# Coolzyh/Globecom2020-ResourceAllocationGNN

Hardware: AMD Instinct MI355X
Metric: graph-instances/sec (fwd+bwd), 20-V2V-link graphs, batch 4096 (higher is better)
Workload: dtype f32; 1 GPU; BASELINE.json configs[1]: 20 V2V links, feat_dim=64, 2-layer GNN, global batch 4096 synthetic graphs cut into 1 shard(s), fit step = fwd+Huber+bwd+Adam; weights=per-node (reference semantics), global_batch=4096, graphs_per_gpu=4096, scaling=strong, n_params=767040, aggregation=edge-bitset-walk, ranks_seen=1, launch=eager, parallelism=dp1

## Files before the change

globecom2020-resourceallocationgnn_amd/csrc/kernels.hpp:

```cpp
#pragma once
#include <hip/hip_runtime.h>
#include <stdint.h>
#include <type_traits>

namespace v2x {

typedef float f32x4 __attribute__((ext_vector_type(4)));
typedef const __attribute__((address_space(1))) float* gfloat_p;
#define V2X_MFMA(a, b, c) __builtin_amdgcn_mfma_f32_16x16x4f32((a), (b), (c), 0, 0, 0)

constexpr int XE = 16;
constexpr int H1 = 80, H2 = 40, H3 = 20;
constexpr int H2P = 48, H3P = 32, CP = 16;
constexpr int LD1 = H1 + 4, LD2 = H2P + 4, LD3 = H3P + 4, LD4 = CP + 4;

struct RowPad { int pad_at, n_pad, k_real; };
__device__ __forceinline__ int real_row(const RowPad& p, int rp) {
  int rr = rp < p.pad_at ? rp : (rp < p.pad_at + p.n_pad ? -1 : rp - p.n_pad);
  return rr < p.k_real ? rr : -1;
}

template <int KP, int NP>
struct WeightImageRegs { float4 v[(KP * (NP / 4) + 255) / 256]; };

// ... 1223 lines not shown
      const int n = col + t;
      df[(((kb * FB + (n >> 4)) * 64) + (n & 15) + 16 * kgp) * 4 + s4] = pv[t];
    }
  }
  if (stage) {
    int ntb = -1;
    if (kp < F) ntb = kp >> 4;
    else if (kp >= F + XE) ntb = FB + ((kp - F - XE) >> 4);
    if (ntb >= 0) {
      float* db = k.bwd + ((int64_t)(stage - 1) * k.S + slot) * (FB * 2 * FB * 256);
      *reinterpret_cast<float4*>(db + ((((col >> 4) * 2 * FB + ntb) * 64) + (kp & 15) + 16 * ((col & 15) >> 2)) * 4) = p;
    }
  }
}

struct AdamArgs {
  AdamPack pack;
  float* param; float* grad; float* mom; float* vel;
  const float* slab; int64_t slab_stride; int n_slabs;
  int n_layers; int64_t layer_end4[16]; int layer_slabs[16];
  int64_t n4;
  float lr_t, beta1, beta2, eps;
  int do_adam;
  int n_adam_blocks;
  const float* rowloss; float* loss; int loss_n_idx, loss_stride; float loss_scale;
  int64_t loss_slot_stride;
  int loss_split; float* loss_part; unsigned* loss_cnt;
  int64_t range_begin4, range_end4;
  int64_t range2_begin4, range2_end4;
  const float* grad_direct;
  int groups;
};

__global__ __launch_bounds__(256) void k_reduce_adam(AdamArgs a) {
  if ((int)blockIdx.x >= a.n_adam_blocks) {
    __shared__ float red[256];
    __shared__ int is_last;
    const int lb = blockIdx.x - a.n_adam_blocks;
    const int slot = lb / a.loss_split, part = lb - slot * a.loss_split;
    const int per = (a.loss_n_idx + a.loss_split - 1) / a.loss_split;
    const int i1 = min((part + 1) * per, a.loss_n_idx);
    float s = 0.f;
    for (int i = part * per + threadIdx.x; i < i1; i += 256) s += a.rowloss[(int64_t)i * a.loss_stride + (int64_t)slot * a.loss_slot_stride];
    red[threadIdx.x] = s;
    __syncthreads();
    for (int o = 128; o > 0; o >>= 1) {
      if ((int)threadIdx.x < o) red[threadIdx.x] += red[threadIdx.x + o];
// ... 7 lines not shown
      __hip_atomic_store(a.loss_part + part, red[0], __ATOMIC_RELAXED, __HIP_MEMORY_SCOPE_AGENT);
      const unsigned ticket = __hip_atomic_fetch_add(a.loss_cnt, 1u, __ATOMIC_ACQ_REL, __HIP_MEMORY_SCOPE_AGENT);
      is_last = ticket == (unsigned)a.loss_split - 1;
      if (is_last) {
        float t = 0.f;
        for (int k = 0; k < a.loss_split; ++k) t += __hip_atomic_load(a.loss_part + k, __ATOMIC_RELAXED, __HIP_MEMORY_SCOPE_AGENT);
        a.loss[slot] = t * a.loss_scale;
        __hip_atomic_store(a.loss_cnt, 0u, __ATOMIC_RELAXED, __HIP_MEMORY_SCOPE_AGENT);
      }
    }
    return;
  }
  __shared__ float4 part[256];
  const int G = a.groups, cols = 256 / G;
  const int col = threadIdx.x % cols, grp = threadIdx.x / cols;
  const int64_t len1 = a.range_end4 - a.range_begin4, len_all = len1 + (a.range2_end4 - a.range2_begin4);
  for (int64_t base = (int64_t)blockIdx.x * cols; base < len_all; base += (int64_t)a.n_adam_blocks * cols) {
    const int64_t t = base + col;
    const bool act = t < len_all;
    const int64_t i = t < len1 ? a.range_begin4 + t : a.range2_begin4 + (t - len1);
    float4 g = make_float4(0.f, 0.f, 0.f, 0.f);
    bool direct = false;
    if (a.slab) {
      if (act) {
        int l = 0;
        while (l + 1 < a.n_layers && i >= a.layer_end4[l]) ++l;
        const int ns = a.layer_slabs[l];
        float4 g1 = make_float4(0.f, 0.f, 0.f, 0.f), g2 = g1, g3 = g1;
        int c = grp;
        for (; c + 3 * G < ns; c += 4 * G) {
          const float4 t0 = reinterpret_cast<const float4*>(a.slab + (int64_t)c * a.slab_stride)[i];
          const float4 t1 = reinterpret_cast<const float4*>(a.slab + (int64_t)(c + G) * a.slab_stride)[i];
          const float4 t2 = reinterpret_cast<const float4*>(a.slab + (int64_t)(c + 2 * G) * a.slab_stride)[i];
          const float4 t3 = reinterpret_cast<const float4*>(a.slab + (int64_t)(c + 3 * G) * a.slab_stride)[i];
          g.x += t0.x; g.y += t0.y; g.z += t0.z; g.w += t0.w;
          g1.x += t1.x; g1.y += t1.y; g1.z += t1.z; g1.w += t1.w;
          g2.x += t2.x; g2.y += t2.y; g2.z += t2.z; g2.w += t2.w;
          g3.x += t3.x; g3.y += t3.y; g3.z += t3.z; g3.w += t3.w;
        }
        for (; c < ns; c += G) {
          const float4 t = reinterpret_cast<const float4*>(a.slab + (int64_t)c * a.slab_stride)[i];
          g.x += t.x; g.y += t.y; g.z += t.z; g.w += t.w;
        }
        g.x = (g.x + g1.x) + (g2.x + g3.x); g.y = (g.y + g1.y) + (g2.y + g3.y);
        g.z = (g.z + g1.z) + (g2.z + g3.z); g.w = (g.w + g1.w) + (g2.w + g3.w);
        if (ns == 0 && grp == 0) g = reinterpret_cast<const float4*>(a.grad_direct)[i];
        direct = ns == 0 && a.grad == a.grad_direct;
      }
      if (G > 1) {
        part[threadIdx.x] = g;
        __syncthreads();
        if (grp == 0) {
          for (int k = 1; k < G; ++k) {
            const float4 t = part[k * cols + col];
            g.x += t.x; g.y += t.y; g.z += t.z; g.w += t.w;
          }
        }
        __syncthreads();
      }
      if (act && grp == 0 && !direct) reinterpret_cast<float4*>(a.grad)[i] = g;
    } else if (act && grp == 0) {
      g = reinterpret_cast<const float4*>(a.grad)[i];
    }
    if (a.do_adam && act && grp == 0) {
      float4 m = reinterpret_cast<float4*>(a.mom)[i], v = reinterpret_cast<float4*>(a.vel)[i];
      float4 p = reinterpret_cast<float4*>(a.param)[i];
      const float b1 = a.beta1, b2 = a.beta2, ob1 = 1.f - a.beta1, ob2 = 1.f - a.beta2;
      m.x = b1 * m.x + ob1 * g.x; m.y = b1 * m.y + ob1 * g.y; m.z = b1 * m.z + ob1 * g.z; m.w = b1 * m.w + ob1 * g.w;
      v.x = b2 * v.x + ob2 * (g.x * g.x); v.y = b2 * v.y + ob2 * (g.y * g.y);
      v.z = b2 * v.z + ob2 * (g.z * g.z); v.w = b2 * v.w + ob2 * (g.w * g.w);
      p.x -= a.lr_t * m.x / (sqrtf(v.x) + a.eps); p.y -= a.lr_t * m.y / (sqrtf(v.y) + a.eps);
      p.z -= a.lr_t * m.z / (sqrtf(v.z) + a.eps); p.w -= a.lr_t * m.w / (sqrtf(v.w) + a.eps);
      reinterpret_cast<float4*>(a.mom)[i] = m;
      reinterpret_cast<float4*>(a.vel)[i] = v;
      reinterpret_cast<float4*>(a.param)[i] = p;
      if (a.pack.fwd) pack_scatter(a.pack, 4 * i, p);
    }
  }
}

__global__ __launch_bounds__(256) void k_zero_rows(float* dst, int64_t slot_stride, int64_t count) {
  float* p = dst + blockIdx.y * slot_stride;
  for (int64_t i = ((int64_t)blockIdx.x * 256 + threadIdx.x) * 4; i < count; i += (int64_t)gridDim.x * 1024)
    *reinterpret_cast<float4*>(p + i) = make_float4(0.f, 0.f, 0.f, 0.f);
}

__global__ __launch_bounds__(256) void k_adam_scalar(float* p, const float* g, float* m, float* v,
// ... 317 lines not shown
```

globecom2020-resourceallocationgnn_amd/csrc/kernels_mlpwg.hpp:

```cpp
#pragma once
#include "kernels.hpp"
#include <type_traits>

namespace v2x {

struct MlpWgLayer { int64_t layer_off, slot_stride; int n_real; RowPad pad; };
struct MlpWgArgs {
  float* slab; int64_t slab_stride; MlpWgLayer l[4];
  int tiles_per_slot, slot_span, tiles_per_wg, n_slots, n_slabs;
  long long* ts;
};
struct MlpTrainWgArgs { MlpArgs a; MlpWgArgs w; };

template <int F>
struct MlpWgLds {
  static constexpr int KB1 = 2 * (F / 16) + 1;
  static constexpr int BLK = 256;
  static constexpr int PER_WAVE = (KB1 + 5 + 5) * BLK;
  static constexpr int STAGE = (MlpLds<F>::TOTAL + 3) / 4 * 4;
  static constexpr int T0 = 0, T1 = KB1 * 5, T2 = T1 + 5 * 3, T3 = T2 + 3 * 2, TILES = T3 + 2;
  static constexpr int NBIAS = (5 + 3 + 2 + 1) * 16;
  static constexpr int TOTAL = STAGE + 4 * PER_WAVE;
  static constexpr int X_SET = TILES * 256;
  static constexpr int X_BIAS = 2 * X_SET;
  static_assert(X_BIAS + 4 * NBIAS <= TOTAL, "accumulator exchange must fit");
};

#define V2X_WAVE_SYNC()                                      \
  do {                                                       \
    __builtin_amdgcn_fence(__ATOMIC_RELEASE, "wavefront");   \
    __builtin_amdgcn_wave_barrier();                         \
    __builtin_amdgcn_fence(__ATOMIC_ACQUIRE, "wavefront");   \
    __builtin_amdgcn_sched_barrier(0);                       \
  } while (0)

#define V2X_DS_ILV(NLD, PER)                                   \
  {                                                            \
    _Pragma("unroll") for (int u_ = 0; u_ < (NLD); ++u_) {     \
      __builtin_amdgcn_sched_group_barrier(0x100, 1, 0);       \
// ... 401 lines not shown
  __syncthreads();
  mark();
  if ((wv & 1) == 0) add(std::false_type{}); else add(std::true_type{});
  const float* bq = sBias4 + min((int)threadIdx.x, G::NBIAS - 1);
  const float bsum4 = (bq[0] + bq[G::NBIAS]) + (bq[2 * G::NBIAS] + bq[3 * G::NBIAS]);
  __syncthreads();
  if (threadIdx.x < G::NBIAS) sBias4[threadIdx.x] = bsum4;
  __syncthreads();
  mark();
  const float* sA = smem;
  const float* sB = smem + G::X_SET;
  const float* sBias = sBias4;
  const int first_wg = tile0 / w.tiles_per_wg;
  const int my_slab = blockIdx.x - first_wg;
  float* slab = w.slab + (int64_t)my_slab * w.slab_stride;
  if constexpr (WG0)
    wg_write<5, H1>(sA + G::T0 * 256, sB + G::T0 * 256, sBias, slab + w.l[0].layer_off + slot * w.l[0].slot_stride, w.l[0]);
  wg_write<3, H2>(sA + G::T1 * 256, sB + G::T1 * 256, sBias + 5 * 16, slab + w.l[1].layer_off + slot * w.l[1].slot_stride, w.l[1]);
  wg_write<2, H3>(sA + G::T2 * 256, sB + G::T2 * 256, sBias + 8 * 16, slab + w.l[2].layer_off + slot * w.l[2].slot_stride, w.l[2]);
  wg_write<1, 0>(sA + G::T3 * 256, sB + G::T3 * 256, sBias + 10 * 16, slab + w.l[3].layer_off + slot * w.l[3].slot_stride, w.l[3]);
  mark();
  if (tsp && tsn < 64) tsp[tsn] = (long long)wall_clock64();
}

}
```

globecom2020-resourceallocationgnn_amd/csrc/knobs.hpp:

```cpp
#pragma once
#include <cstdlib>

namespace v2x {

struct Knobs {
  int fused = 1;
  int fused_compl = 1;
  int fused_split = -1;
  int fused_split_fwd = 1;
  int fused_split_bwd = 1;
  int fused_ts = 0;
  int small_predict = 1;
  int small_pinned = 1;
  int ragged_fused = 1;
  int ragged_fused_bwd = 1;
  int ragged_packed = 1;
  int ragged_plan_fold = 1;
  int ragged_small = 0;
  int frag_handoff = 1;
  int frag_with_dense0_role = 1;
  int mlp_wg0 = -1;
  int mlp_wg0_tiles = 12;
  int dqn_fused_targets = 1;
  int wide_merge = 1;
  int wide_fold = 1;
  int wide_adam = 1;
  int wide_tail = 1;
  int wide_slots = 0;
  int wg_embed_merge = 1;
  int wg_rounds = 0;
  int wg_chunk = 0;
  int wg_chunk_gnn = 0;
  int wg_chunk_dense = 1024;
  int wg_chunk_embed = 0;
  int wg_chunk_d123 = 512;
  int wg_chunk_merged = 0;
  int wg_merged_min_rows = 64;
// ... 17 lines not shown
  num("V2X_FUSED_SPLIT", k.fused_split);
  num("V2X_FUSED_SPLIT_FWD", k.fused_split_fwd);
  num("V2X_FUSED_SPLIT_BWD", k.fused_split_bwd);
  num("V2X_FUSED_TS", k.fused_ts);
  num("V2X_SMALL_PREDICT", k.small_predict);
  num("V2X_SMALL_PINNED", k.small_pinned);
  num("V2X_RAGGED_FUSED", k.ragged_fused);
  num("V2X_RAGGED_FUSED_BWD", k.ragged_fused_bwd);
  num("V2X_RAGGED_PACKED", k.ragged_packed);
  num("V2X_RAGGED_PLAN_FOLD", k.ragged_plan_fold);
  num("V2X_RAGGED_SMALL", k.ragged_small);
  num("V2X_FRAG_HANDOFF", k.frag_handoff);
  num("V2X_FRAG_WITH_DENSE0_ROLE", k.frag_with_dense0_role);
  num("V2X_MLP_WG0", k.mlp_wg0);
  num("V2X_MLP_WG0_TILES", k.mlp_wg0_tiles);
  num("V2X_DQN_FUSED_TARGETS", k.dqn_fused_targets);
  num("V2X_WIDE_MERGE", k.wide_merge);
  num("V2X_WIDE_FOLD", k.wide_fold);
  num("V2X_WIDE_ADAM", k.wide_adam);
  num("V2X_WIDE_TAIL", k.wide_tail);
  num("V2X_WIDE_SLOTS", k.wide_slots);
  num("V2X_WG_EMBED_MERGE", k.wg_embed_merge);
  num("V2X_WG_ROUNDS", k.wg_rounds);
  num("V2X_WG_CHUNK", k.wg_chunk);
  num("V2X_WG_CHUNK_GNN", k.wg_chunk_gnn);
  num("V2X_WG_CHUNK_DENSE", k.wg_chunk_dense);
  num("V2X_WG_CHUNK_EMBED", k.wg_chunk_embed);
  num("V2X_WG_CHUNK_D123", k.wg_chunk_d123);
  num("V2X_WG_CHUNK_MERGED", k.wg_chunk_merged);
  num("V2X_WG_MERGED_MIN_ROWS", k.wg_merged_min_rows);
// ... 19 lines not shown
```

globecom2020-resourceallocationgnn_amd/csrc/v2xgnn.hip:

```cpp
#include "../../include/v2xgnn.h"
#include "kernels.hpp"
#include "kernels_wide.hpp"
#include "kernels_fused.hpp"
#include "kernels_fused_split.hpp"
#include "kernels_mlpwg.hpp"
#include "kernels_small.hpp"
#include "kernels_ragged.hpp"
#include "kernels_ragged_small.hpp"
#include "host_pack.hpp"
#include "knobs.hpp"

#include <hip/hip_runtime.h>
#include <algorithm>
#include <cmath>
#include <cstdio>
#include <cstdlib>
#include <cstring>
#include <map>
#include <mutex>
#include <string>
#include <type_traits>
#include <vector>

using namespace v2x;

namespace {

thread_local std::string g_err;

struct LayerDesc {
  int64_t off;
  int64_t slot_stride;
  int k_real, n_out;
  int kp, np;
  RowPad pad;
  int n_slabs = 0;
};

struct DevBuf {
  void* p = nullptr;
  size_t cap = 0;
};

struct ProfRec { int id; hipEvent_t ev0, ev1; };

struct GraphKey {
  int kind; const void* ptrs[12]; int sizes[6]; double scalar;
  int64_t gen;
  bool operator<(const GraphKey& o) const { return memcmp(this, &o, sizeof(GraphKey)) < 0; }
};

// ... 10 lines not shown
  int64_t iterations = 0;
  int64_t cap_rows = 0;
  std::vector<float*> h, a;
  float *z1 = nullptr, *z2 = nullptr, *z3 = nullptr, *q = nullptr;
  float *dq = nullptr, *dz1 = nullptr, *dz2 = nullptr, *dz3 = nullptr, *gha = nullptr, *rowloss = nullptr;
  std::vector<float*> dpre;
  unsigned* nbmask = nullptr;
  bool frag_live = false;
  unsigned short* gate_bits = nullptr;
  int64_t gate_stride = 0;
  hipStream_t cap = nullptr;
  float* loss_dev = nullptr;
  float* loss_part = nullptr;
  float* zero_buf = nullptr;
  float* slab = nullptr; int slab_cap = 0;
  int reduce_groups = 0;
  std::vector<int32_t> wide_rec_tiles, wide_rec_roles;
  DevBuf st_xe, st_nbr, st_goff, st_rp, st_ci, st_y, st_q;
  DevBuf adj_mask;
  DevBuf plan_buf;
  int plan_len = 0;
  Knobs knobs;
  long long* ts_buf = nullptr;
  bool raw_params = false;
  bool pk_stale = false;
  unsigned long long* small_h = nullptr;
  unsigned long long* small_sync = nullptr;
  char* pin_h = nullptr; char* pin_d = nullptr;
  float *pk_fwd = nullptr, *pk_bwd = nullptr;
  unsigned long long* xchg_buf = nullptr;
  unsigned long long* xchg_sync = nullptr;
  int xchg_cap_tiles = 0;
  int* flag_host = nullptr;
  int* flag_dev = nullptr;
  bool have_fwd = false;
  std::string err;
  bool prof = false;
  std::vector<std::string> prof_names;
  std::vector<ProfRec> prof_recs;
  struct GraphEntry { hipGraphExec_t exec; std::vector<int> n_slabs; bool frag_live; int reduce_groups; };
  int64_t ws_gen = 0;
  std::map<GraphKey, GraphEntry> graphs;
  bool capturing = false;
  float* adam_scal = nullptr;
  bool prof_no_fuse = false;
  hipStream_t dp_st = nullptr;
  std::vector<hipEvent_t> dp_ev;
};

namespace {

#define FAIL(m, code, ...)                                   \
  do {                                                       \
    char _b[512];                                            \
    snprintf(_b, sizeof(_b), __VA_ARGS__);                   \
// ... 191 lines not shown
  } else {
    nc = (n_idx + rows - 1) / rows;
  }
  if (nc < 1) nc = 1;
  const int max_nc = (n_idx + 4 * WG_TR - 1) / (4 * WG_TR);
  if (nc > max_nc) nc = max_nc;
  if (nc < 1) nc = 1;
  int chunk = (n_idx + nc - 1) / nc;
  chunk = (chunk + 4 * WG_TR - 1) / (4 * WG_TR) * (4 * WG_TR);
  nc = (n_idx + chunk - 1) / chunk;
  if (nc < 1) nc = 1;
  *chunk_out = chunk;
  return nc;
}

int ensure_slabs(v2x_model* m, int nc) {
  if (nc <= m->slab_cap) return V2X_OK;
  if (m->capturing) FAIL(m, V2X_ESTATE, "slab growth during graph capture");
  drop_graphs(m);
  if (m->slab) HIPCHK(m, hipFree(m->slab));
  m->slab = nullptr;
  HIPCHK(m, hipMalloc(reinterpret_cast<void**>(&m->slab), (size_t)nc * m->P * sizeof(float)));
  HIPCHK(m, hipMemset(m->slab, 0, (size_t)nc * m->P * sizeof(float)));
  HIPCHK(m, hipDeviceSynchronize());
  m->slab_cap = nc;
  return V2X_OK;
}

struct FlagWord { int* host = nullptr; int* dev = nullptr; };
int alloc_flag(FlagWord* f) {
  void* h = nullptr;
  if (hipHostMalloc(&h, 64, hipHostMallocMapped) != hipSuccess) return V2X_EHIP;
  memset(h, 0, 64);
  void* d = nullptr;
  if (hipHostGetDevicePointer(&d, h, 0) != hipSuccess) { hipHostFree(h); return V2X_EHIP; }
  f->host = (int*)h; f->dev = (int*)d;
  return V2X_OK;
}
// ... 549 lines not shown
  s.n_slabs = gx;
  return s;
}

template <int F>
int launch_mlp_train_wg_f(v2x_model* m, hipStream_t st, const MlpArgs& a, int n_slots, bool wg0) {
  const size_t lds = (size_t)MlpWgLds<F>::TOTAL * 4;
  const MlpWgSplit sp = mlp_wg_split(a.n_idx, n_slots);
  if (sp.n_slabs > m->slab_cap) FAIL(m, V2X_ESTATE, "mlp_train_wg: slabs not pre-sized (%d > %d)", sp.n_slabs, m->slab_cap);
  MlpTrainWgArgs t;
  memset(&t, 0, sizeof(t));
  t.a = a;
  t.w.slab = m->slab; t.w.slab_stride = m->P;
  t.w.tiles_per_slot = sp.tiles_per_slot; t.w.slot_span = sp.slot_span; t.w.tiles_per_wg = sp.tiles_per_wg; t.w.n_slots = n_slots; t.w.n_slabs = sp.n_slabs;
  t.w.ts = m->ts_buf ? m->ts_buf + 2 * 8 * 64 : nullptr;
  for (int i = 0; i < 4; ++i) {
    LayerDesc& ld = m->dense[i];
    ld.n_slabs = sp.n_slabs;
    t.w.l[i] = MlpWgLayer{ld.off, ld.slot_stride, ld.n_out, ld.pad};
  }
  if constexpr (F == 64) {
    if (!wg0) {
      if (a.frag_groups > 0) { auto k = k_mlp_train_wg<F, true, false>; LAUNCH(m, "k_mlp_train_wg123", k, dim3(sp.n_wgs), 256, lds, st, t); }
      else { auto k = k_mlp_train_wg<F, false, false>; LAUNCH(m, "k_mlp_train_wg123", k, dim3(sp.n_wgs), 256, lds, st, t); }
      return V2X_OK;
    }
  }
  if (!wg0) FAIL(m, V2X_ESTATE, "mlp_train_wg: Dense-0 outside the launch needs feat_dim 64");
  if (a.frag_groups > 0) { auto k = k_mlp_train_wg<F, true>; LAUNCH(m, "k_mlp_train_wg", k, dim3(sp.n_wgs), 256, lds, st, t); }
  else { auto k = k_mlp_train_wg<F>; LAUNCH(m, "k_mlp_train_wg", k, dim3(sp.n_wgs), 256, lds, st, t); }
  return V2X_OK;
}

// ... 34 lines not shown

int layer_work(const LayerDesc& ld) { return (ld.kp / 16) * (ld.np / 16); }

int wgrad_role(v2x_model* m, LayerDesc& ld, int kind, const IdxMap& x, int total_work, const WgSeg* segs, int n_seg,
               const float* dpre, int d_stride, WgradArgs& a, int rows_override = 0) {
  int chunk;
  const bool gnn_kind = kind < WG_KIND_DENSE0 || kind >= WG_KIND_EMBED_NONBR;
  const Knobs& kn = m->knobs;
  const int rows_dense = kn.wg_chunk_dense, rows_embed = kn.wg_chunk_embed;
  int rows_g = kn.wg_chunk_gnn > 0 ? kn.wg_chunk_gnn : (is_wide(m) ? 1024 : 896);
  if (rows_embed > 0 && (kind == WG_KIND_EMBED || kind == WG_KIND_EMBED_NONBR)) rows_g = rows_embed;
  if (rows_override > 0) rows_g = rows_override;
  const int nc = role_chunks(kn, x.n_idx, x.grid_y, layer_work(ld), total_work, &chunk, (gnn_kind || rows_override > 0) ? rows_g : rows_dense);
  if (nc > m->slab_cap) FAIL(m, V2X_ESTATE, "wgrad: slabs not pre-sized (%d > %d)", nc, m->slab_cap);
  ld.n_slabs = nc;
  memset(&a, 0, sizeof(a));
  for (int i = 0; i < n_seg; ++i) a.seg[i] = segs[i];
  a.n_seg = n_seg;
  a.dpre = dpre; a.d_stride = d_stride; a.n_real = ld.n_out;
  a.kp = ld.kp; a.np = ld.np; a.pad = ld.pad;
  a.slab = m->slab; a.slab_stride = m->P; a.layer_off = ld.off; a.slot_stride = ld.slot_stride;
  a.n_idx = x.n_idx; a.row_stride = x.row_stride; a.base_mul = x.base_mul; a.chunk = chunk;
  a.idx_base = x.idx_base; a.chunk_base = 0; a.n_chunks = nc; a.kind = kind;
  a.dpre_slot_major = (kind >= WG_KIND_DENSE1 && kind <= WG_KIND_DENSE3) ? 1 : 0;
  a.srow_stride = (int)srow_stride(m);
  a.zeros = m->zero_buf;
  a.ts = (m->ts_buf && (kind == WG_KIND_GNN || kind >= WG_KIND_GNN_E1)) ? m->ts_buf + 3 * 8 * 64 : nullptr;
  return V2X_OK;
}

// ... 207 lines not shown
    for (auto* v : {&m->gnn, &m->dense})
      for (const LayerDesc& ld : *v) {
        a.layer_end4[nl] = (ld.off + ld.slot_stride * m->S) / 4;
        a.layer_slabs[nl] = ld.n_slabs;
        ++nl;
      }
    a.n_layers = nl;
  }
  a.n4 = m->P / 4;
  a.range_begin4 = bucket_begin(m, bucket) / 4; a.range_end4 = bucket_end(m, bucket) / 4;
  if (range_begin >= 0) { a.range_begin4 = range_begin / 4; a.range_end4 = range_end / 4; }
  if (fused_adam) {
    a.range_begin4 = 0; a.range_end4 = m->gnn[1].off / 4;
    a.range2_begin4 = m->dense[1].off / 4; a.range2_end4 = m->P / 4;
  }
  a.do_adam = do_adam ? 1 : 0;
  if (do_adam) {
    if (advance_iteration) m->iterations += 1;
    a.lr_t = adam_lr_t(m, m->iterations);
    a.beta1 = m->cfg.beta1; a.beta2 = m->cfg.beta2; a.eps = m->cfg.eps;
    if (m->pk_fwd) { a.pack.fwd = m->pk_fwd; a.pack.bwd = m->pk_bwd; a.pack.F = m->F; a.pack.S = m->S; a.pack.L = m->L; a.pack.xr = m->Dn + m->De; }
  }
  int max_slabs_used = 0;
  for (int l = 0; l < a.n_layers; ++l) max_slabs_used = std::max(max_slabs_used, a.layer_slabs[l]);
  a.groups = 1;
  if (a.slab && a.n4 < 256 * 1024 && max_slabs_used >= 16) a.groups = a.n4 < 64 * 1024 ? 16 : 4;
  m->reduce_groups = a.groups;
  const int cols = 256 / a.groups;
  int blocks = (int)((a.range_end4 - a.range_begin4 + a.range2_end4 - a.range2_begin4 + cols - 1) / cols);
  if (blocks > 2048) blocks = 2048;
  if (blocks < 1) blocks = 1;
  a.n_adam_blocks = blocks;
  a.rowloss = m->rowloss; a.loss = m->loss_dev; a.loss_n_idx = lj.n_idx; a.loss_stride = lj.stride; a.loss_scale = lj.scale; a.loss_slot_stride = lj.slot_stride;
  a.grad_direct = m->grads;
  a.loss_split = (lj.n_out == 1 && lj.n_idx > 16384) ? 64 : 1;
  a.loss_part = m->loss_part; a.loss_cnt = reinterpret_cast<unsigned*>(m->loss_part + 64);
  LAUNCH(m, do_adam ? (n_slabs > 0 ? "k_reduce_adam" : "k_adam") : "k_grad_reduce", k_reduce_adam,
         dim3(blocks + lj.n_out * a.loss_split), 256, 0, st, a);
  return V2X_OK;
}

LossJob loss_job(const v2x_model* m, const DevBatch& d, int n_global) {
  const float inv = 1.0f / (float)((double)n_global * m->C);
  if (m->cfg.variable_graphs) return LossJob{1, d.R, 1, inv, 0};
// ... 440 lines not shown
    HIPCHK(m, hipMemcpyAsync(loss_out, m->loss_dev, n * sizeof(float), hipMemcpyDeviceToHost, st));
    HIPCHK(m, hipStreamSynchronize(st));
    CHK(check_flag(m));
  }
  return V2X_OK;
}

template <typename Body>
int run_maybe_graph(v2x_model* m, hipStream_t& st, const GraphKey& key, Body body) {
  const bool want = m->cfg.use_graph && !m->prof && st != nullptr;
  if (!want) return body();
  auto it = m->graphs.find(key);
  if (it != m->graphs.end()) {
    size_t i = 0;
    for (auto* v : {&m->gnn, &m->dense})
      for (LayerDesc& ld : *v) ld.n_slabs = it->second.n_slabs[i++];
    m->frag_live = it->second.frag_live;
    m->reduce_groups = it->second.reduce_groups;
    HIPCHK(m, hipGraphLaunch(it->second.exec, st));
    return V2X_OK;
  }
  hipGraph_t g = nullptr;
  hipStream_t const user = st, cap = m->cap ? m->cap : st;
  HIPCHK(m, hipStreamBeginCapture(cap, hipStreamCaptureModeThreadLocal));
  m->capturing = true;
  st = cap;
  const int r = body();
  st = user;
  m->capturing = false;
  hipError_t e = hipStreamEndCapture(cap, &g);
  if (r != V2X_OK) { if (g) hipGraphDestroy(g); return r; }
  if (e != hipSuccess) FAIL(m, V2X_EHIP, "hipStreamEndCapture: %s", hipGetErrorString(e));
  hipGraphExec_t ge = nullptr;
  e = hipGraphInstantiate(&ge, g, nullptr, nullptr, 0);
  hipGraphDestroy(g);
  if (e != hipSuccess) FAIL(m, V2X_EHIP, "hipGraphInstantiate: %s", hipGetErrorString(e));
  if (m->graphs.size() >= 16) drop_graphs(m);
  v2x_model::GraphEntry entry;
  entry.exec = ge;
  entry.frag_live = m->frag_live;
  entry.reduce_groups = m->reduce_groups;
  for (auto* v : {&m->gnn, &m->dense})
    for (const LayerDesc& ld : *v) entry.n_slabs.push_back(ld.n_slabs);
  m->graphs[key] = entry;
  HIPCHK(m, hipGraphLaunch(ge, st));
  return V2X_OK;
}

GraphKey make_key(int kind, const DevBatch& d, const void* y, int n_global) {
  GraphKey k;
  memset(&k, 0, sizeof(k));
  k.kind = kind;
  k.ptrs[0] = d.xe; k.ptrs[1] = d.nbr; k.ptrs[2] = d.goff; k.ptrs[3] = d.rp; k.ptrs[4] = d.ci; k.ptrs[5] = y;
  k.sizes[0] = d.B; k.sizes[1] = d.R; k.sizes[2] = d.E; k.sizes[3] = d.max_nodes; k.sizes[4] = d.max_edges;
  k.sizes[5] = n_global;
  return k;
}

// ... 128 lines not shown
    m->flag_host = f.host; m->flag_dev = f.dev;
  }
  if (hipStreamCreateWithFlags(&m->cap, hipStreamNonBlocking) != hipSuccess) return fail("capture stream");
  if (hipDeviceSynchronize() != hipSuccess) return fail("synchronisation");
  *out = m;
  return V2X_OK;
}

void v2x_destroy(v2x_model* m) {
  if (!m) return;
  hipSetDevice(m->cfg.device);
  hipDeviceSynchronize();
  for (auto& kv : m->graphs) hipGraphExecDestroy(kv.second.exec);
  for (auto& r : m->prof_recs) { hipEventDestroy(r.ev0); hipEventDestroy(r.ev1); }
  float* ptrs[] = {m->params, m->grads, m->mom, m->vel, m->z1, m->z2, m->z3, m->q, m->dq, m->dz1, m->dz2, m->dz3,
                   m->gha, m->rowloss, m->loss_dev, m->slab, m->zero_buf, m->loss_part, m->pk_fwd, m->pk_bwd, m->adam_scal};
  for (float* p : m->dpre) if (p) hipFree(p);
  if (m->gate_bits) hipFree(m->gate_bits);
  if (m->nbmask) hipFree(m->nbmask);
  for (auto& e : m->dp_ev) if (e) hipEventDestroy(e);
  if (m->dp_st) hipStreamDestroy(m->dp_st);
  if (m->cap) hipStreamDestroy(m->cap);
  for (float* p : ptrs) if (p) hipFree(p);
  for (float* p : m->h) if (p) hipFree(p);
  for (float* p : m->a) if (p) hipFree(p);
  DevBuf* bufs[] = {&m->st_xe, &m->st_nbr, &m->st_goff, &m->st_rp, &m->st_ci, &m->st_y, &m->st_q, &m->adj_mask, &m->plan_buf};
  for (DevBuf* b : bufs) if (b->p) hipFree(b->p);
  if (m->flag_host) hipHostFree(m->flag_host);
  if (m->ts_buf) hipFree(m->ts_buf);
  if (m->small_h) hipFree(m->small_h);
  if (m->xchg_sync) {
// ... 703 lines not shown
  if (!m || !out) FAIL(m, V2X_EINVAL, "null argument");
  if (!m->ts_buf) FAIL(m, V2X_ESTATE, "phase stamps need V2X_FUSED_TS=1 when the model is created");
  HIPCHK(m, hipDeviceSynchronize());
  HIPCHK(m, hipMemcpy(out, m->ts_buf, (size_t)std::min(n, 4 * 8 * 64) * 8, hipMemcpyDeviceToHost));
  return V2X_OK;
}

int v2x_debug_ragged_plan(v2x_model* m, int32_t* out, int n) {
  if (!m || !out || n < 0) FAIL(m, V2X_EINVAL, "null argument");
  if (!m->plan_buf.p || m->plan_len <= 0) FAIL(m, V2X_ESTATE, "no ragged fused forward has run on this model");
  HIPCHK(m, hipDeviceSynchronize());
  HIPCHK(m, hipMemcpy(out, m->plan_buf.p, (size_t)std::min(n, m->plan_len) * 4, hipMemcpyDeviceToHost));
  return m->plan_len;
}

int v2x_debug_layer_slabs(v2x_model* m, int32_t* out, int n) {
  if (!m || !out || n < 0) FAIL(m, V2X_EINVAL, "null argument");
  const int want = (int)(m->gnn.size() + m->dense.size()) + 1;
  if (n < want) FAIL(m, V2X_EINVAL, "layer_slabs: room for %d values needed", want);
  HIPCHK(m, hipDeviceSynchronize());
  int k = 0;
  for (auto* v : {&m->gnn, &m->dense})
    for (const LayerDesc& ld : *v) out[k++] = ld.n_slabs;
  out[k++] = m->reduce_groups;
  return k;
}

int v2x_wide_tiling_plan(int32_t n_idx, int32_t grid_z, int32_t n_out, int32_t slots, int32_t tail, int32_t out[4]) {
  v2x_model* m = nullptr;
  if (!out) FAIL(m, V2X_EINVAL, "wide_tiling_plan: null output");
// ... 57 lines not shown
```

globecom2020-resourceallocationgnn_amd/lib.py:

```python
import ctypes as C
import os

_HERE = os.path.dirname(os.path.abspath(__file__))
_LIB = None

V2X_OK = 0
V2X_EINVAL = -1
V2X_ECOMM = -5
V2X_EBUDGET = -6

V2X_DP_ALLREDUCE, V2X_DP_BUCKETS, V2X_DP_SHARDED = 0, 1, 2


class V2XError(RuntimeError):
    pass


class V2XInvalidArgument(V2XError, ValueError):
    """V2X_EINVAL: a library error (V2XError) and the exception class Keras raises on bad inputs (ValueError)."""


class V2XCommError(V2XError):
    """V2X_ECOMM: a collective of the v2x_comm table failed (the text names it and its bucket)."""

# ... 177 lines not shown
    ("v2x_comm_rccl_unique_id", C.c_int, [_P]),
    ("v2x_comm_rccl_create", C.c_int, [_P, _I, _I, _I, C.POINTER(Comm)]),
    ("v2x_comm_rccl_destroy", C.c_int, [C.POINTER(Comm)]),
    ("v2x_train_step_dp", C.c_int, [_P, C.POINTER(Batch), _P, C.c_int, _I, C.POINTER(Comm), C.c_int, _P, C.c_int, _P]),
    ("v2x_dqn_step_dp", C.c_int, [_P, _P, C.POINTER(Batch), C.POINTER(Batch), _P, _P, C.c_double, C.c_int32, C.POINTER(Comm),
                                  _P, _P, C.c_int, _P]),
    ("v2x_pack_feed", C.c_int, [C.POINTER(Feed), C.c_int, _P, _P, _P, _P, _P]),
    ("v2x_validate_batch", C.c_int, [_P, C.POINTER(Batch), _I, _P]),
    ("v2x_check_errors", C.c_int, [_P, _P]),
    ("v2x_reset_exchange", C.c_int, [_P]),
    ("v2x_debug_exchange_counters", _P, [_P]),
    ("v2x_debug_split_counters", _P, [_P, C.POINTER(C.c_int32)]),
    ("v2x_debug_phase_stamps", C.c_int, [_P, _P, C.c_int]),
    ("v2x_debug_ragged_plan", C.c_int, [_P, _P, C.c_int]),
    ("v2x_debug_layer_slabs", C.c_int, [_P, _P, C.c_int]),
    ("v2x_wide_tiling_plan", C.c_int, [_I, _I, _I, _I, _I, C.POINTER(_I)]),
    ("v2x_debug_wide_tiling", C.c_int, [_P, _P, C.c_int]),
    ("v2x_profile_enable", C.c_int, [_P, C.c_int]),
    ("v2x_path_info", C.c_int, [_P, _P, C.c_char_p, C.c_int]),
    ("v2x_profile_read", C.c_int, [_P, C.c_char_p, C.c_int, C.POINTER(C.c_double), C.POINTER(_L), C.c_int]),
    ("v2x_opt_workspace_bytes", _L, [C.POINTER(OptProblem)]),
    ("v2x_opt_search", C.c_int, [C.POINTER(OptProblem), _P, _P, _P, _P]),
    ("v2x_opt_rewards", C.c_int, [C.POINTER(OptProblem), _P, _L, _L, _P, _P]),
    ("v2x_opt_landscape_workspace_bytes", _L, [C.POINTER(OptProblem), C.c_int32]),
    ("v2x_opt_landscape", C.c_int, [C.POINTER(OptProblem), _P, _P, C.c_int32, _P, _P, _P]),
    ("v2x_opt_bound_workspace_bytes", _L, [C.POINTER(OptProblem), _L]),
    ("v2x_opt_search_bound", C.c_int, [C.POINTER(OptProblem), _P, _L, _P, _P, C.POINTER(_L), _P]),
    ("v2x_opt_search_bound_seeded", C.c_int, [C.POINTER(OptProblem), _P, _L, _P, _P, _P, C.POINTER(_L), _P]),
    ("v2x_opt_count_bound_workspace_bytes", _L, [C.POINTER(OptProblem), C.c_int32, _L]),
    ("v2x_opt_count_bound", C.c_int, [C.POINTER(OptProblem), _P, _P, C.c_int32, _L, _P, _P, _P, _P, C.POINTER(_L), _P]),
# ... 84 lines not shown
```

include/v2xgnn.h:

```cpp
#ifndef V2XGNN_H
#define V2XGNN_H

#include <stdint.h>

#ifdef __cplusplus
extern "C" {
#endif

#define V2X_OK            0
#define V2X_EINVAL       -1
#define V2X_EHIP         -2
#define V2X_ENOMEM       -3
#define V2X_ESTATE       -4
#define V2X_ECOMM        -5
#define V2X_EBUDGET      -6

#define V2X_XE_WIDTH     16

typedef struct v2x_model v2x_model;

typedef struct v2x_config {
  int32_t n_nodes;
  int32_t n_channels;
  int32_t feat_dim;
// ... 405 lines not shown

typedef struct v2x_eval_sweep {
  v2x_eval_mixed base;
  int32_t K, pad_;
  v2x_model* const* models;
  float* q;
} v2x_eval_sweep;
int64_t v2x_eval_sweep_result_bytes(int32_t E, int32_t n, int32_t rb, int32_t T, int32_t schemes);
int  v2x_eval_sweep_mixed(const v2x_eval_sweep* s, const v2x_traj_ws* ws , void* stream);

int  v2x_profile_enable(v2x_model* m, int enable);
int  v2x_path_info(v2x_model* m, const v2x_batch* b, char* out, int cap);
int  v2x_debug_phase_stamps(v2x_model* m, int64_t* out, int n);
int  v2x_debug_ragged_plan(v2x_model* m, int32_t* out, int n);
int  v2x_debug_layer_slabs(v2x_model* m, int32_t* out, int n);
int  v2x_wide_tiling_plan(int32_t n_idx, int32_t grid_z, int32_t n_out, int32_t slots, int32_t tail, int32_t out[4]);
int  v2x_debug_wide_tiling(v2x_model* m, int32_t* out, int n);
int  v2x_profile_read(v2x_model* m, char* names_out, int names_cap, double* ms_out, int64_t* calls_out,
                      int max_entries);

#ifdef __cplusplus
}
#endif
#endif
```

Before: 16.16 million graph-instances/s.

## Store dense-layer weight-gradient slabs in fragment-major layout and scatter in Adam

The MLP weight-gradient workgroups now dump their MFMA accumulator tiles straight into a fragment-major slab buffer with contiguous float4 stores, replacing the per-layer row-major wg_write remapping. The reduce/Adam kernel gains a fragment range that sums these slabs with coalesced float4 loads and then maps each fragment element back to its parameter index, doing scalar gathers and scatters for grad, momentum, variance and param. The aim is cheaper, coalesced slab writes in the wgrad epilogue. The cost is uncoalesced scalar parameter accesses in Adam, an extra slab buffer, and more index arithmetic. It is on by default through a new knob.

Result: no change. 16.14 million graph-instances/s (-0.1%).

```diff
diff --git a/globecom2020-resourceallocationgnn_amd/csrc/kernels.hpp b/globecom2020-resourceallocationgnn_amd/csrc/kernels.hpp
--- a/globecom2020-resourceallocationgnn_amd/csrc/kernels.hpp
+++ b/globecom2020-resourceallocationgnn_amd/csrc/kernels.hpp
@@ -1261,6 +1261,34 @@
   }
 }
 
+struct DenseFragLayer { int64_t off; int slot_stride, n_real, nt, tile0, bias0, on; RowPad pad; };
+
+__device__ __forceinline__ void dense_frag_targets(const DenseFragLayer* fl, int n_tiles_all, int slot, int f, int64_t (&e)[4]) {
+  e[0] = e[1] = e[2] = e[3] = -1;
+  if (f >= n_tiles_all * 64) {
+    const int b = (f - n_tiles_all * 64) * 4 + n_tiles_all * 256;
+    int d = 0;
+    while (d < 3 && b >= fl[d + 1].bias0) ++d;
+    const int n = b - fl[d].bias0;
+    if (fl[d].on && n < fl[d].n_real) {
+      e[0] = fl[d].off + (int64_t)slot * fl[d].slot_stride + (int64_t)fl[d].pad.k_real * fl[d].n_real + n;
+      e[1] = e[0] + 1; e[2] = e[0] + 2; e[3] = e[0] + 3;
+    }
+    return;
+  }
+  const int tile = f >> 6, lane = f & 63;
+  int d = 0;
+  while (d < 3 && tile >= fl[d + 1].tile0) ++d;
+  const DenseFragLayer& l = fl[d];
+  const int tl = tile - l.tile0, kt = tl / l.nt, n = (tl - kt * l.nt) * 16 + (lane & 15);
+  if (!l.on || n >= l.n_real) return;
+#pragma unroll
+  for (int r = 0; r < 4; ++r) {
+    const int rr = real_row(l.pad, kt * 16 + (lane >> 4) * 4 + r);
+    if (rr >= 0) e[r] = l.off + (int64_t)slot * l.slot_stride + (int64_t)rr * l.n_real + n;
+  }
+}
+
 struct AdamArgs {
   AdamPack pack;
   float* param; float* grad; float* mom; float* vel;
@@ -1277,7 +1305,29 @@
   int64_t range2_begin4, range2_end4;
   const float* grad_direct;
   int groups;
+  const float* slab_frag; int64_t frag_slab_stride; int frag_slot_stride, frag_slots, frag_items, frag_f0, frag_tiles, frag_slabs;
+  DenseFragLayer frag[4];
 };
+
+__device__ __forceinline__ void adam_1(const AdamArgs& a, float g, float& m, float& v, float& p) {
+  const float b1 = a.beta1, b2 = a.beta2, ob1 = 1.f - a.beta1, ob2 = 1.f - a.beta2;
+  m = __builtin_fmaf(b1, m, ob1 * g);
+  v = __builtin_fmaf(b2, v, ob2 * (g * g));
+  p -= a.lr_t * m / (sqrtf(v) + a.eps);
+}
+
+__device__ __forceinline__ void adam_update_scatter(const AdamArgs& a, const int64_t (&e)[4], float4 g4, float (&m)[4], float (&v)[4], float (&p)[4]) {
+  const float g[4] = {g4.x, g4.y, g4.z, g4.w};
+#pragma unroll
+  for (int r = 0; r < 4; ++r)
+    if (e[r] >= 0) {
+      a.grad[e[r]] = g[r];
+      if (a.do_adam) {
+        adam_1(a, g[r], m[r], v[r], p[r]);
+        a.mom[e[r]] = m[r]; a.vel[e[r]] = v[r]; a.param[e[r]] = p[r];
+      }
+    }
+}
 
 __global__ __launch_bounds__(256) void k_reduce_adam(AdamArgs a) {
   if ((int)blockIdx.x >= a.n_adam_blocks) {
@@ -1315,37 +1365,61 @@
   __shared__ float4 part[256];
   const int G = a.groups, cols = 256 / G;
   const int col = threadIdx.x % cols, grp = threadIdx.x / cols;
-  const int64_t len1 = a.range_end4 - a.range_begin4, len_all = len1 + (a.range2_end4 - a.range2_begin4);
+  const int64_t len1 = a.range_end4 - a.range_begin4, len12 = len1 + (a.range2_end4 - a.range2_begin4);
+  const int64_t len_all = len12 + (int64_t)a.frag_slots * a.frag_items;
   for (int64_t base = (int64_t)blockIdx.x * cols; base < len_all; base += (int64_t)a.n_adam_blocks * cols) {
     const int64_t t = base + col;
     const bool act = t < len_all;
+    const bool fragc = act && t >= len12;
     const int64_t i = t < len1 ? a.range_begin4 + t : a.range2_begin4 + (t - len1);
+    const int fslot = fragc ? (int)((t - len12) / a.frag_items) : 0;
+    const int ff = fragc ? a.frag_f0 + (int)((t - len12) - (int64_t)fslot * a.frag_items) : 0;
     float4 g = make_float4(0.f, 0.f, 0.f, 0.f);
     bool direct = false;
+    const bool upd = a.do_adam && act && grp == 0;
+    float4 m4 = g, v4 = g, p4 = g;
+    int64_t fe[4] = {-1, -1, -1, -1};
+    float fm[4], fv[4], fp[4];
+    if (fragc && grp == 0) {
+      dense_frag_targets(a.frag, a.frag_tiles, fslot, ff, fe);
+      if (a.do_adam) {
+#pragma unroll
+        for (int r = 0; r < 4; ++r) {
+          const int64_t x = fe[r] >= 0 ? fe[r] : 0;
+          fm[r] = a.mom[x]; fv[r] = a.vel[x]; fp[r] = a.param[x];
+        }
+      }
+    } else if (upd) {
+      m4 = reinterpret_cast<const float4*>(a.mom)[i]; v4 = reinterpret_cast<const float4*>(a.vel)[i];
+      p4 = reinterpret_cast<const float4*>(a.param)[i];
+    }
     if (a.slab) {
       if (act) {
         int l = 0;
         while (l + 1 < a.n_layers && i >= a.layer_end4[l]) ++l;
-        const int ns = a.layer_slabs[l];
+        const int ns = fragc ? a.frag_slabs : a.layer_slabs[l];
+        const float4* src4 = fragc ? reinterpret_cast<const float4*>(a.slab_frag + (int64_t)fslot * a.frag_slot_stride) + ff
+                                   : reinterpret_cast<const float4*>(a.slab) + i;
+        const int64_t stride4 = (fragc ? a.frag_slab_stride : a.slab_stride) / 4;
         float4 g1 = make_float4(0.f, 0.f, 0.f, 0.f), g2 = g1, g3 = g1;
         int c = grp;
         for (; c + 3 * G < ns; c += 4 * G) {
-          const float4 t0 = reinterpret_cast<const float4*>(a.slab + (int64_t)c * a.slab_stride)[i];
-          const float4 t1 = reinterpret_cast<const float4*>(a.slab + (int64_t)(c + G) * a.slab_stride)[i];
-          const float4 t2 = reinterpret_cast<const float4*>(a.slab + (int64_t)(c + 2 * G) * a.slab_stride)[i];
-          const float4 t3 = reinterpret_cast<const float4*>(a.slab + (int64_t)(c + 3 * G) * a.slab_stride)[i];
+          const float4 t0 = src4[(int64_t)c * stride4];
+          const float4 t1 = src4[(int64_t)(c + G) * stride4];
+          const float4 t2 = src4[(int64_t)(c + 2 * G) * stride4];
+          const float4 t3 = src4[(int64_t)(c + 3 * G) * stride4];
           g.x += t0.x; g.y += t0.y; g.z += t0.z; g.w += t0.w;
           g1.x += t1.x; g1.y += t1.y; g1.z += t1.z; g1.w += t1.w;
           g2.x += t2.x; g2.y += t2.y; g2.z += t2.z; g2.w += t2.w;
           g3.x += t3.x; g3.y += t3.y; g3.z += t3.z; g3.w += t3.w;
         }
         for (; c < ns; c += G) {
-          const float4 t = reinterpret_cast<const float4*>(a.slab + (int64_t)c * a.slab_stride)[i];
+          const float4 t = src4[(int64_t)c * stride4];
           g.x += t.x; g.y += t.y; g.z += t.z; g.w += t.w;
         }
         g.x = (g.x + g1.x) + (g2.x + g3.x); g.y = (g.y + g1.y) + (g2.y + g3.y);
         g.z = (g.z + g1.z) + (g2.z + g3.z); g.w = (g.w + g1.w) + (g2.w + g3.w);
-        if (ns == 0 && grp == 0) g = reinterpret_cast<const float4*>(a.grad_direct)[i];
+        if (ns == 0 && grp == 0 && !fragc) g = reinterpret_cast<const float4*>(a.grad_direct)[i];
         direct = ns == 0 && a.grad == a.grad_direct;
       }
       if (G > 1) {
@@ -1359,19 +1433,18 @@
         }
         __syncthreads();
       }
+      if (fragc) {
+        if (grp == 0) adam_update_scatter(a, fe, g, fm, fv, fp);
+        continue;
+      }
       if (act && grp == 0 && !direct) reinterpret_cast<float4*>(a.grad)[i] = g;
     } else if (act && grp == 0) {
       g = reinterpret_cast<const float4*>(a.grad)[i];
     }
-    if (a.do_adam && act && grp == 0) {
-      float4 m = reinterpret_cast<float4*>(a.mom)[i], v = reinterpret_cast<float4*>(a.vel)[i];
-      float4 p = reinterpret_cast<float4*>(a.param)[i];
-      const float b1 = a.beta1, b2 = a.beta2, ob1 = 1.f - a.beta1, ob2 = 1.f - a.beta2;
-      m.x = b1 * m.x + ob1 * g.x; m.y = b1 * m.y + ob1 * g.y; m.z = b1 * m.z + ob1 * g.z; m.w = b1 * m.w + ob1 * g.w;
-      v.x = b2 * v.x + ob2 * (g.x * g.x); v.y = b2 * v.y + ob2 * (g.y * g.y);
-      v.z = b2 * v.z + ob2 * (g.z * g.z); v.w = b2 * v.w + ob2 * (g.w * g.w);
-      p.x -= a.lr_t * m.x / (sqrtf(v.x) + a.eps); p.y -= a.lr_t * m.y / (sqrtf(v.y) + a.eps);
-      p.z -= a.lr_t * m.z / (sqrtf(v.z) + a.eps); p.w -= a.lr_t * m.w / (sqrtf(v.w) + a.eps);
+    if (upd) {
+      float4 m = m4, v = v4, p = p4;
+      adam_1(a, g.x, m.x, v.x, p.x); adam_1(a, g.y, m.y, v.y, p.y);
+      adam_1(a, g.z, m.z, v.z, p.z); adam_1(a, g.w, m.w, v.w, p.w);
       reinterpret_cast<float4*>(a.mom)[i] = m;
       reinterpret_cast<float4*>(a.vel)[i] = v;
       reinterpret_cast<float4*>(a.param)[i] = p;
diff --git a/globecom2020-resourceallocationgnn_amd/csrc/kernels_mlpwg.hpp b/globecom2020-resourceallocationgnn_amd/csrc/kernels_mlpwg.hpp
--- a/globecom2020-resourceallocationgnn_amd/csrc/kernels_mlpwg.hpp
+++ b/globecom2020-resourceallocationgnn_amd/csrc/kernels_mlpwg.hpp
@@ -9,6 +9,7 @@
   float* slab; int64_t slab_stride; MlpWgLayer l[4];
   int tiles_per_slot, slot_span, tiles_per_wg, n_slots, n_slabs;
   long long* ts;
+  float* slab_frag; int64_t frag_slab_stride; int frag_slot_stride, frag;
 };
 struct MlpTrainWgArgs { MlpArgs a; MlpWgArgs w; };
 
@@ -23,6 +24,7 @@
   static constexpr int TOTAL = STAGE + 4 * PER_WAVE;
   static constexpr int X_SET = TILES * 256;
   static constexpr int X_BIAS = 2 * X_SET;
+  static constexpr int FRAG_SLOT = TILES * 256 + NBIAS;
   static_assert(X_BIAS + 4 * NBIAS <= TOTAL, "accumulator exchange must fit");
 };
 
@@ -454,11 +456,23 @@
   const int first_wg = tile0 / w.tiles_per_wg;
   const int my_slab = blockIdx.x - first_wg;
   float* slab = w.slab + (int64_t)my_slab * w.slab_stride;
-  if constexpr (WG0)
-    wg_write<5, H1>(sA + G::T0 * 256, sB + G::T0 * 256, sBias, slab + w.l[0].layer_off + slot * w.l[0].slot_stride, w.l[0]);
-  wg_write<3, H2>(sA + G::T1 * 256, sB + G::T1 * 256, sBias + 5 * 16, slab + w.l[1].layer_off + slot * w.l[1].slot_stride, w.l[1]);
-  wg_write<2, H3>(sA + G::T2 * 256, sB + G::T2 * 256, sBias + 8 * 16, slab + w.l[2].layer_off + slot * w.l[2].slot_stride, w.l[2]);
-  wg_write<1, 0>(sA + G::T3 * 256, sB + G::T3 * 256, sBias + 10 * 16, slab + w.l[3].layer_off + slot * w.l[3].slot_stride, w.l[3]);
+  if (w.frag) {
+    float* fs = w.slab_frag + (int64_t)my_slab * w.frag_slab_stride + (int64_t)slot * w.frag_slot_stride;
+    const float4* a4 = reinterpret_cast<const float4*>(sA);
+    const float4* b4 = reinterpret_cast<const float4*>(sB);
+    float4* d4 = reinterpret_cast<float4*>(fs);
+    for (int f = TB * 64 + (int)threadIdx.x; f < G::TILES * 64; f += 256) {
+      const float4 u = a4[f], v = b4[f];
+      d4[f] = make_float4(u.x + v.x, u.y + v.y, u.z + v.z, u.w + v.w);
+    }
+    if (threadIdx.x < G::NBIAS) fs[G::TILES * 256 + threadIdx.x] = sBias[threadIdx.x];
+  } else {
+    if constexpr (WG0)
+      wg_write<5, H1>(sA + G::T0 * 256, sB + G::T0 * 256, sBias, slab + w.l[0].layer_off + slot * w.l[0].slot_stride, w.l[0]);
+    wg_write<3, H2>(sA + G::T1 * 256, sB + G::T1 * 256, sBias + 5 * 16, slab + w.l[1].layer_off + slot * w.l[1].slot_stride, w.l[1]);
+    wg_write<2, H3>(sA + G::T2 * 256, sB + G::T2 * 256, sBias + 8 * 16, slab + w.l[2].layer_off + slot * w.l[2].slot_stride, w.l[2]);
+    wg_write<1, 0>(sA + G::T3 * 256, sB + G::T3 * 256, sBias + 10 * 16, slab + w.l[3].layer_off + slot * w.l[3].slot_stride, w.l[3]);
+  }
   mark();
   if (tsp && tsn < 64) tsp[tsn] = (long long)wall_clock64();
 }
diff --git a/globecom2020-resourceallocationgnn_amd/csrc/knobs.hpp b/globecom2020-resourceallocationgnn_amd/csrc/knobs.hpp
--- a/globecom2020-resourceallocationgnn_amd/csrc/knobs.hpp
+++ b/globecom2020-resourceallocationgnn_amd/csrc/knobs.hpp
@@ -21,6 +21,7 @@
   int frag_with_dense0_role = 1;
   int mlp_wg0 = -1;
   int mlp_wg0_tiles = 12;
+  int dense_slab_frag = 1;
   int dqn_fused_targets = 1;
   int wide_merge = 1;
   int wide_fold = 1;
@@ -68,6 +69,7 @@
   num("V2X_FRAG_WITH_DENSE0_ROLE", k.frag_with_dense0_role);
   num("V2X_MLP_WG0", k.mlp_wg0);
   num("V2X_MLP_WG0_TILES", k.mlp_wg0_tiles);
+  num("V2X_DENSE_SLAB_FRAG", k.dense_slab_frag);
   num("V2X_DQN_FUSED_TARGETS", k.dqn_fused_targets);
   num("V2X_WIDE_MERGE", k.wide_merge);
   num("V2X_WIDE_FOLD", k.wide_fold);
diff --git a/globecom2020-resourceallocationgnn_amd/csrc/v2xgnn.hip b/globecom2020-resourceallocationgnn_amd/csrc/v2xgnn.hip
--- a/globecom2020-resourceallocationgnn_amd/csrc/v2xgnn.hip
+++ b/globecom2020-resourceallocationgnn_amd/csrc/v2xgnn.hip
@@ -35,6 +35,7 @@
   int kp, np;
   RowPad pad;
   int n_slabs = 0;
+  bool slab_frag = false;
 };
 
 struct DevBuf {
@@ -75,6 +76,7 @@
   float* loss_part = nullptr;
   float* zero_buf = nullptr;
   float* slab = nullptr; int slab_cap = 0;
+  float* slab_frag = nullptr;
   int reduce_groups = 0;
   std::vector<int32_t> wide_rec_tiles, wide_rec_roles;
   DevBuf st_xe, st_nbr, st_goff, st_rp, st_ci, st_y, st_q;
@@ -99,7 +101,7 @@
   bool prof = false;
   std::vector<std::string> prof_names;
   std::vector<ProfRec> prof_recs;
-  struct GraphEntry { hipGraphExec_t exec; std::vector<int> n_slabs; bool frag_live; int reduce_groups; };
+  struct GraphEntry { hipGraphExec_t exec; std::vector<int> n_slabs; std::vector<char> slab_frag; bool frag_live; int reduce_groups; };
   int64_t ws_gen = 0;
   std::map<GraphKey, GraphEntry> graphs;
   bool capturing = false;
@@ -321,14 +323,32 @@
   return nc;
 }
 
+int dense_frag_slot_floats(const v2x_model* m) {
+  switch (m->F) {
+    case 16: return MlpWgLds<16>::FRAG_SLOT;
+    case 32: return MlpWgLds<32>::FRAG_SLOT;
+    case 64: return MlpWgLds<64>::FRAG_SLOT;
+  }
+  return 0;
+}
+int64_t frag_slab_stride(const v2x_model* m) { return (int64_t)m->S * dense_frag_slot_floats(m); }
+
 int ensure_slabs(v2x_model* m, int nc) {
   if (nc <= m->slab_cap) return V2X_OK;
   if (m->capturing) FAIL(m, V2X_ESTATE, "slab growth during graph capture");
   drop_graphs(m);
   if (m->slab) HIPCHK(m, hipFree(m->slab));
   m->slab = nullptr;
+  if (m->slab_frag) HIPCHK(m, hipFree(m->slab_frag));
+  m->slab_frag = nullptr;
+  m->slab_cap = 0;
   HIPCHK(m, hipMalloc(reinterpret_cast<void**>(&m->slab), (size_t)nc * m->P * sizeof(float)));
   HIPCHK(m, hipMemset(m->slab, 0, (size_t)nc * m->P * sizeof(float)));
+  if (m->knobs.dense_slab_frag && frag_slab_stride(m) > 0) {
+    const size_t fb = (size_t)nc * frag_slab_stride(m) * sizeof(float);
+    HIPCHK(m, hipMalloc(reinterpret_cast<void**>(&m->slab_frag), fb));
+    HIPCHK(m, hipMemset(m->slab_frag, 0, fb));
+  }
   HIPCHK(m, hipDeviceSynchronize());
   m->slab_cap = nc;
   return V2X_OK;
@@ -908,9 +928,13 @@
   t.w.slab = m->slab; t.w.slab_stride = m->P;
   t.w.tiles_per_slot = sp.tiles_per_slot; t.w.slot_span = sp.slot_span; t.w.tiles_per_wg = sp.tiles_per_wg; t.w.n_slots = n_slots; t.w.n_slabs = sp.n_slabs;
   t.w.ts = m->ts_buf ? m->ts_buf + 2 * 8 * 64 : nullptr;
+  const bool frag = m->slab_frag != nullptr;
+  t.w.frag = frag ? 1 : 0;
+  t.w.slab_frag = m->slab_frag; t.w.frag_slab_stride = frag_slab_stride(m); t.w.frag_slot_stride = MlpWgLds<F>::FRAG_SLOT;
   for (int i = 0; i < 4; ++i) {
     LayerDesc& ld = m->dense[i];
     ld.n_slabs = sp.n_slabs;
+    ld.slab_frag = frag && (i > 0 || wg0);
     t.w.l[i] = MlpWgLayer{ld.off, ld.slot_stride, ld.n_out, ld.pad};
   }
   if constexpr (F == 64) {
@@ -975,6 +999,7 @@
   const int nc = role_chunks(kn, x.n_idx, x.grid_y, layer_work(ld), total_work, &chunk, (gnn_kind || rows_override > 0) ? rows_g : rows_dense);
   if (nc > m->slab_cap) FAIL(m, V2X_ESTATE, "wgrad: slabs not pre-sized (%d > %d)", nc, m->slab_cap);
   ld.n_slabs = nc;
+  ld.slab_frag = false;
   memset(&a, 0, sizeof(a));
   for (int i = 0; i < n_seg; ++i) a.seg[i] = segs[i];
   a.n_seg = n_seg;
@@ -1212,6 +1237,25 @@
     a.range_begin4 = 0; a.range_end4 = m->gnn[1].off / 4;
     a.range2_begin4 = m->dense[1].off / 4; a.range2_end4 = m->P / 4;
   }
+  if (n_slabs > 0 && m->slab_frag && m->dense[1].slab_frag) {
+    const int d0 = m->dense[0].slab_frag ? 0 : 1;
+    const int64_t fb4 = m->dense[d0].off / 4;
+    if (a.range_end4 > fb4) {
+      if (a.range_end4 != m->P / 4 || a.range_begin4 > fb4 || a.range2_end4 != a.range2_begin4)
+        FAIL(m, V2X_ESTATE, "slab sum: a range that cuts through the fragment-major Dense slabs");
+      a.range_end4 = fb4;
+      a.slab_frag = m->slab_frag; a.frag_slab_stride = frag_slab_stride(m); a.frag_slot_stride = dense_frag_slot_floats(m);
+      a.frag_tiles = (a.frag_slot_stride - 11 * 16) / 256;
+      int tile0 = 0, bias0 = a.frag_tiles * 256;
+      for (int i = 0; i < 4; ++i) {
+        const LayerDesc& ld = m->dense[i];
+        a.frag[i] = DenseFragLayer{ld.off, (int)ld.slot_stride, ld.n_out, ld.np / 16, tile0, bias0, ld.slab_frag ? 1 : 0, ld.pad};
+        tile0 += (ld.kp / 16) * (ld.np / 16); bias0 += ld.np;
+      }
+      a.frag_slots = m->S; a.frag_f0 = a.frag[d0].tile0 * 64; a.frag_items = a.frag_slot_stride / 4 - a.frag_f0;
+      a.frag_slabs = m->dense[1].n_slabs;
+    }
+  }
   a.do_adam = do_adam ? 1 : 0;
   if (do_adam) {
     if (advance_iteration) m->iterations += 1;
@@ -1225,7 +1269,7 @@
   if (a.slab && a.n4 < 256 * 1024 && max_slabs_used >= 16) a.groups = a.n4 < 64 * 1024 ? 16 : 4;
   m->reduce_groups = a.groups;
   const int cols = 256 / a.groups;
-  int blocks = (int)((a.range_end4 - a.range_begin4 + a.range2_end4 - a.range2_begin4 + cols - 1) / cols);
+  int blocks = (int)((a.range_end4 - a.range_begin4 + a.range2_end4 - a.range2_begin4 + (int64_t)a.frag_slots * a.frag_items + cols - 1) / cols);
   if (blocks > 2048) blocks = 2048;
   if (blocks < 1) blocks = 1;
   a.n_adam_blocks = blocks;
@@ -1696,7 +1740,7 @@
   if (it != m->graphs.end()) {
     size_t i = 0;
     for (auto* v : {&m->gnn, &m->dense})
-      for (LayerDesc& ld : *v) ld.n_slabs = it->second.n_slabs[i++];
+      for (LayerDesc& ld : *v) { ld.n_slabs = it->second.n_slabs[i]; ld.slab_frag = it->second.slab_frag[i] != 0; ++i; }
     m->frag_live = it->second.frag_live;
     m->reduce_groups = it->second.reduce_groups;
     HIPCHK(m, hipGraphLaunch(it->second.exec, st));
@@ -1723,7 +1767,7 @@
   entry.frag_live = m->frag_live;
   entry.reduce_groups = m->reduce_groups;
   for (auto* v : {&m->gnn, &m->dense})
-    for (const LayerDesc& ld : *v) entry.n_slabs.push_back(ld.n_slabs);
+    for (const LayerDesc& ld : *v) { entry.n_slabs.push_back(ld.n_slabs); entry.slab_frag.push_back(ld.slab_frag ? 1 : 0); }
   m->graphs[key] = entry;
   HIPCHK(m, hipGraphLaunch(ge, st));
   return V2X_OK;
@@ -1882,7 +1926,7 @@
   for (auto& kv : m->graphs) hipGraphExecDestroy(kv.second.exec);
   for (auto& r : m->prof_recs) { hipEventDestroy(r.ev0); hipEventDestroy(r.ev1); }
   float* ptrs[] = {m->params, m->grads, m->mom, m->vel, m->z1, m->z2, m->z3, m->q, m->dq, m->dz1, m->dz2, m->dz3,
-                   m->gha, m->rowloss, m->loss_dev, m->slab, m->zero_buf, m->loss_part, m->pk_fwd, m->pk_bwd, m->adam_scal};
+                   m->gha, m->rowloss, m->loss_dev, m->slab, m->slab_frag, m->zero_buf, m->loss_part, m->pk_fwd, m->pk_bwd, m->adam_scal};
   for (float* p : m->dpre) if (p) hipFree(p);
   if (m->gate_bits) hipFree(m->gate_bits);
   if (m->nbmask) hipFree(m->nbmask);
@@ -2616,6 +2660,12 @@
   return m->plan_len;
 }
 
+int v2x_debug_dense_slab_layout(v2x_model* m, int32_t* out, int n) {
+  if (!m || !out || n < 4) FAIL(m, V2X_EINVAL, "dense_slab_layout: room for 4 values needed");
+  for (int i = 0; i < 4; ++i) out[i] = m->dense[i].slab_frag ? 1 : 0;
+  return 4;
+}
+
 int v2x_debug_layer_slabs(v2x_model* m, int32_t* out, int n) {
   if (!m || !out || n < 0) FAIL(m, V2X_EINVAL, "null argument");
   const int want = (int)(m->gnn.size() + m->dense.size()) + 1;
diff --git a/globecom2020-resourceallocationgnn_amd/lib.py b/globecom2020-resourceallocationgnn_amd/lib.py
--- a/globecom2020-resourceallocationgnn_amd/lib.py
+++ b/globecom2020-resourceallocationgnn_amd/lib.py
@@ -215,6 +215,7 @@
     ("v2x_debug_phase_stamps", C.c_int, [_P, _P, C.c_int]),
     ("v2x_debug_ragged_plan", C.c_int, [_P, _P, C.c_int]),
     ("v2x_debug_layer_slabs", C.c_int, [_P, _P, C.c_int]),
+    ("v2x_debug_dense_slab_layout", C.c_int, [_P, _P, C.c_int]),
     ("v2x_wide_tiling_plan", C.c_int, [_I, _I, _I, _I, _I, C.POINTER(_I)]),
     ("v2x_debug_wide_tiling", C.c_int, [_P, _P, C.c_int]),
     ("v2x_profile_enable", C.c_int, [_P, C.c_int]),
diff --git a/include/v2xgnn.h b/include/v2xgnn.h
--- a/include/v2xgnn.h
+++ b/include/v2xgnn.h
@@ -443,6 +443,7 @@
 int  v2x_debug_phase_stamps(v2x_model* m, int64_t* out, int n);
 int  v2x_debug_ragged_plan(v2x_model* m, int32_t* out, int n);
 int  v2x_debug_layer_slabs(v2x_model* m, int32_t* out, int n);
+int  v2x_debug_dense_slab_layout(v2x_model* m, int32_t* out, int n);
 int  v2x_wide_tiling_plan(int32_t n_idx, int32_t grid_z, int32_t n_out, int32_t slots, int32_t tail, int32_t out[4]);
 int  v2x_debug_wide_tiling(v2x_model* m, int32_t* out, int n);
 int  v2x_profile_read(v2x_model* m, char* names_out, int names_cap, double* ms_out, int64_t* calls_out,
```
